# AiRyunn/BoT

Measured on AMD Instinct MI355X. Metric: edges/sec full-batch GAT fwd+bwd on ogbn-arxiv; achieved HBM GB/s vs peak, higher is better.
Workload: dtype f32

## Files before the change

bot_amd/_C.py:

```python
from __future__ import annotations

import ctypes
import os
from ctypes import c_char_p, c_double, c_float, c_int32, c_int64, c_uint64, c_void_p

import torch

_HERE = os.path.dirname(os.path.abspath(__file__))
LIB_PATH = os.environ.get("BOT_AMD_LIB") or os.path.join(_HERE, "lib", "libbot_gnn.so")
ABI_VERSION = 19

if not os.path.exists(LIB_PATH):
    raise ImportError(
        f"{LIB_PATH} is missing: build the gfx950 kernels first "
        "(`make -C bot_amd/csrc` or `python -c 'import __graft_entry__ as g; g.build()'`). "
        "bot_amd has no CPU / PyTorch fallback."
    )
_lib = ctypes.CDLL(LIB_PATH)

_P = c_void_p
_SIGS = {
    "bot_abi_version": (ctypes.c_int, []),
    "bot_last_error": (c_char_p, []),
    "bot_last_kernel": (c_char_p, []),
# ... 82 lines not shown
                                                 _P, _P, c_int64, c_int32, c_int32, _P]),
    "bot_bn_act_fwd_f32": (ctypes.c_int, [_P, c_int64, c_int64, c_int32, _P, _P, _P, _P, c_int32, c_float, c_uint64, _P, _P, c_int64, _P]),
    "bot_bn_act_bwd_reduce_f32": (ctypes.c_int, [_P, c_int64, _P, c_int64, c_int64, c_int32, _P, _P, _P, _P, c_int32, c_float,
                                                 c_uint64, _P, _P, _P, _P, _P]),
    "bot_bn_act_bwd_apply_f32": (ctypes.c_int, [_P, c_int64, _P, c_int64, c_int64, c_int32, _P, _P, _P, _P, c_int32, c_float,
                                                c_uint64, _P, _P, _P, c_double, _P, c_int64, _P, _P]),
    "bot_halves_tn_combine_f32": (ctypes.c_int, [_P, _P, c_int32, c_int32, c_int32, c_int32, _P, _P, _P, c_int64, _P]),
    "bot_halves_scale_from_slots2_f32": (ctypes.c_int, [_P, c_float, _P, c_float, _P, _P]),
    "bot_halves_tail_f16": (ctypes.c_int, [c_int64, c_int32, _P, _P, _P, _P, _P, c_int64, c_int32, _P]),
    "bot_spmm_dot_halves_fits": (ctypes.c_int, [_P, c_int64, c_int64, _P, c_int64, c_int64, c_int32, c_int32, _P, c_int64, c_int64, c_int32]),
    "bot_spmm_dot_halves_f16": (ctypes.c_int, [_P, _P, c_int64, c_int64, _P, c_int64, _P, _P, c_int64, _P, c_int64, c_int64, _P, _P, _P, c_int64, c_int64,
                                               c_int32, c_int32, _P, _P, c_int64, c_int64, c_int32, _P, _P, _P]),
    "bot_gemm_halves3_nt_bn_rows": (c_int32, [c_int64]),
    "bot_gemm_halves3_nt3_f32": (ctypes.c_int, [c_int64, c_int64, c_int64, _P, _P, c_int64, _P, _P, c_int64, c_int64, _P, c_int64, c_int64, c_int32, _P, c_int64,
                                                _P, c_int32, _P]),
    "bot_bn_act_bwd_reduce_partials_f32": (ctypes.c_int, [_P, c_int32, c_int32, _P, _P, _P]),
    "bot_bn_bwd_bound_partials_f32": (ctypes.c_int, [c_int32, _P, c_int32, _P, _P, c_double, _P, _P, _P, _P]),
    "bot_bn_bwd_partials_finish_f32": (ctypes.c_int, [_P, _P, c_int32, c_int32, _P, _P, c_int32, c_double, _P, _P, _P, _P]),
    "bot_gemm_halves3_nt2_f32": (ctypes.c_int, [c_int64, c_int64, c_int64, _P, _P, c_int64, _P, _P, c_int64, c_int64, _P, c_int64, c_int64, c_int32, _P, c_int64,
                                                c_int32, _P]),
    "bot_halves_split_frag_f16": (ctypes.c_int, [_P, c_int64, c_int64, c_int32, _P, _P, c_int32, _P]),
    "bot_gemm_halves3_tn2_f32": (ctypes.c_int, [c_int64, c_int64, c_int64, c_int64, c_int64, _P, _P, _P, c_int64, _P, c_int64, c_int64, _P, c_int64, c_int64, _P,
                                                c_int64, _P, c_int32, _P]),
    "bot_stream_create": (ctypes.c_int, [c_int32, _P]),
    "bot_gemm_halves3_nt_grouped2_f32": (ctypes.c_int, [c_int64, c_int64, _P, _P, _P, c_int64, c_int64, _P, c_int64, c_int64, _P, c_int64, c_int32, _P,
                                                        c_int32, _P, _P, c_int32, _P, _P, _P, _P, c_int32, c_int32, _P]),
    "bot_bn_stats_halves_partials_f32": (ctypes.c_int, [_P, _P, c_int32, _P, c_int64, c_int32, c_float, c_float, _P, _P, _P, _P, _P, _P, _P, c_float, _P, _P, _P]),
    "bot_absmax_slots": (c_int32, []),
    "bot_absmax_slots_f32": (ctypes.c_int, [_P, c_int64, c_int64, c_int32, _P, _P]),
    "bot_halves_scale_from_slots_f32": (ctypes.c_int, [_P, _P, _P]),
# ... 735 lines not shown
        sg = torch.empty(self.F, dtype=torch.float32, device=self.x.device)
        sgx = torch.empty(self.F, dtype=torch.float32, device=self.x.device)
        _check(_lib.bot_bn_bwd_partials_finish_f32(self.part.data_ptr(), self.pmax.data_ptr(), self.nblk, self.F, sg.data_ptr(), sgx.data_ptr(),
                                                   int(bool(batch_stats)), float(total_count), _ptr(self.weight), self.invstd.data_ptr(), slots.data_ptr(),
                                                   _stream()), "bn_bwd_partials_finish")
        return sg, sgx

    def bound(self, sum_g, sum_gx, total_count, slots):
        assert self.pmax is not None
        _dev(slots)
        _check(_lib.bot_bn_bwd_bound_partials_f32(self.F, self.pmax.data_ptr(), self.nblk, _ptr(sum_g), _ptr(sum_gx), float(total_count), _ptr(self.weight),
                                                  self.invstd.data_ptr(), slots.data_ptr(), _stream()), "bn_bwd_bound_partials")
        return slots


def gemm_halves3_nt(a, b, scale_a, scale_b, piece_a, piece_b, k, out=None, mode=0, a2_off=None, scale_a2=None, k_split=0, b_frag=False, n=None, bn=None):
    _dev(a, b, scale_a, scale_b, scale_a2)
    m = a.shape[0]
    if n is None:
        assert not b_frag
        n = b.shape[0]
    if out is None:
        out = torch.empty((m, n), dtype=torch.float32, device=a.device)
    st = None
    if bn is not None:
        if not bn.fits(m, n, k):
            raise BotKernelError("gemm_halves3_nt: this product cannot carry the BatchNorm-backward by-product (BnBwdStats.fits)")
        st = bn.struct()
    _check(_timed("gemm_halves", (m, n, 3 * k, 1), lambda: _lib.bot_gemm_halves3_nt3_f32(
        m, n, k, scale_a.data_ptr(), _ptr(scale_a2), int(k_split), scale_b.data_ptr(), a.data_ptr(), _ld(a), 2 * piece_a if a2_off is None else a2_off,
        b.data_ptr(), _ld(b), piece_b, int(bool(b_frag)), out.data_ptr(), _ld(out), ctypes.addressof(st) if st is not None else None, int(mode), _stream())),
        "gemm_halves3_nt")
    return out


def halves_split_frag(x, scale, piece):
    _dev(x, scale)
    x = _mat(x, "x")
    n, F = x.shape
    assert piece % 64 == 0 and piece >= F
    out = torch.empty((2 * ((n + 15) // 16) * (piece // 32), 512), dtype=torch.float16, device=x.device)
    _check(_lib.bot_halves_split_frag_f16(x.data_ptr(), x.stride(0), n, F, _ptr(scale), out.data_ptr(), piece, _stream()), "halves_split_frag")
    return out


def _table(rows, width):
# ... 600 lines not shown
```

bot_amd/csrc/halves3.hip:

```cpp
#include <hip/hip_fp16.h>

#include <stdlib.h>
#include <string.h>

#include <algorithm>
#include <type_traits>
#include <utility>

#include "common.h"

namespace bot {
namespace {

constexpr int BK = 32;

typedef _Float16 half8 __attribute__((ext_vector_type(8)));
typedef float f32x4 __attribute__((ext_vector_type(4)));

struct H3Args {
    const _Float16* A;
    const _Float16* B;
    const float* scale_a;
    const float* scale_b;
    float* C;
// ... 11 lines not shown
    float* stats_minmax;
    float* stats_pivot;
    int stats_F;
    const float* bnb_x;
    int64_t bnb_ldx;
    const float* bnb_mean;
    const float* bnb_invstd;
    const float* bnb_w;
    const float* bnb_b;
    int bnb_relu;
    float bnb_p;
    uint64_t bnb_seed;
    const uint64_t* bnb_seed_offset;
    float* bnb_part;
    float* bnb_pmax;
    int b_frag;
    int mode;
};

struct H3Group {
    int b_row0, n_valid;
    int a_off0, a_off1;
    int k_steps, pad;
    int64_t c_off;
};
constexpr int kMaxGroups = 12;
struct H3Groups {
    H3Group g[kMaxGroups];
    int k_seg;
};
// ... 267 lines not shown
}
template <int N, class F>
__device__ __forceinline__ void static_for(F& f) {
    static_for_impl(f, std::make_integer_sequence<int, N>{});
}

__device__ __forceinline__ half8 load16(const void* tile_base, uint32_t voff, int soff) {
#if defined(__HIP_DEVICE_COMPILE__)
    const __amdgpu_buffer_rsrc_t rsrc = __builtin_amdgcn_make_buffer_rsrc(const_cast<void*>(tile_base), 0, 0x7fffffff, 0x00020000);
    return __builtin_bit_cast(half8, __builtin_amdgcn_raw_buffer_load_b128(rsrc, voff, soff, 0));
#else
    return half8{};
#endif
}

template <bool GROUPED, bool BFRAG, bool BNB = false>
__device__ __forceinline__ void gemm_halves3_nt64_body(const H3Args& p, const H3Groups* groups) {
    static_assert(!(GROUPED && BNB), "the BatchNorm-backward by-product indexes the output columns of a plain launch");
    constexpr int BM = 256, BN = 256, kWaves = 8, MT = BM / 16, NT = BN / kWaves / 16;
    constexpr int kRow = 4 * BK;
    constexpr int kABytes = BM * kRow;
    constexpr int kStageBytes = 2 * kABytes, kStages = 2;
    constexpr int GA = BM / 8 / kWaves;
    static_assert(NT == 2 && GA == 4 && kRow == 128, "wave tile 256 x 32, 128-byte rows");
    __shared__ __attribute__((aligned(1024))) unsigned char lds[kStages * kStageBytes];
    const int tid = threadIdx.x, lane = tid & 63, w = __builtin_amdgcn_readfirstlane(tid >> 6);
    const int b = blockIdx.x, xcd = b & 7, j = b >> 3;
    const int tm = (j / p.tiles_n) * 8 + xcd, tn = j % p.tiles_n;
    if (tm >= p.tiles_m) return;
    const int m0 = tm * BM;
    int n0 = tn * BN, n_valid = p.N - n0, T = p.K / BK, a_off0 = 0, a_off1 = 0, k_seg = 0;
    int64_t c0 = n0;
    if constexpr (GROUPED) {
// ... 5 lines not shown

    const _Float16* tileA = p.A + (int64_t)m0 * p.lda;
    const _Float16* tileB = p.B + (int64_t)n0 * p.ldb;
    uint32_t offA[GA];
#pragma unroll
    for (int h = 0; h < GA; ++h) {
        const int row = (w + kWaves * h) * 8 + (lane >> 3);
        offA[h] = ((uint32_t)(min(m0 + row, p.M - 1) - m0) * (uint32_t)p.lda + (((lane & 7) ^ ((row >> 1) & 7)) * 8)) * 2;
    }
    const int a2b = p.a2_off * 2;
    auto issue_a = [&](int i, int stage, int it) {
        const int q = i / GA, h = i % GA;
        dma16(tileA, lds + stage * kStageBytes + q * kABytes + (w + kWaves * h) * 1024, offA[h],
              (GROUPED ? it * kRow + (2 * it < k_seg ? a_off0 : a_off1) : it * kRow) + q * a2b);
    };
    uint32_t offB[NT];
    int tileoff[NT];
    const int Tk = p.K / BK;
#pragma unroll
    for (int nt = 0; nt < NT; ++nt) {
        if constexpr (BFRAG) {
            offB[nt] = lane * 16;
            tileoff[nt] = min((n0 + w * (NT * 16) + nt * 16) >> 4, ((p.N + 15) >> 4) - 1) * Tk * 1024;
        } else {
            offB[nt] = ((uint32_t)(min(n0 + w * (NT * 16) + nt * 16 + (lane & 15), p.N - 1) - n0) * (uint32_t)p.ldb) * 2 + (lane >> 4) * 16;
            tileoff[nt] = 0;
        }
    }
    const int b2 = BFRAG ? ((p.N + 15) >> 4) * Tk * 1024 : p.b2_off * 2;
    const _Float16* baseB = BFRAG ? p.B : tileB;
// ... 106 lines not shown
    static_assert(32 * P * 4 <= kStages * kStageBytes / kWaves, "staging slab does not fit the wave's share of the LDS");
    float* stg = reinterpret_cast<float*>(lds + w * (kStages * kStageBytes / kWaves));
    const int q4 = (lane >> 4) * 4, l15 = lane & 15, l7 = lane & 7;
    const int col = w * (NT * 16) + l7 * 4;
    float cs[4] = {1.f, 1.f, 1.f, 1.f}, ch[4] = {0.f, 0.f, 0.f, 0.f};
    const bool affine = p.col_scale != nullptr || p.col_shift != nullptr;
    if (affine) {
#pragma unroll
        for (int e = 0; e < 4; ++e)
            if (col + e < n_valid) {
                if (p.col_scale) cs[e] = p.col_scale[c0 + col + e];
                if (p.col_shift) ch[e] = p.col_shift[c0 + col + e];
            }
    }
    float amax = 0.f;
    const bool stats = p.stats_part != nullptr;
    float st_s[4] = {0.f, 0.f, 0.f, 0.f}, st_q[4] = {0.f, 0.f, 0.f, 0.f}, st_mn[4], st_mx[4], piv[4] = {0.f, 0.f, 0.f, 0.f};
#pragma unroll
    for (int e = 0; e < 4; ++e) st_mn[e] = INFINITY, st_mx[e] = -INFINITY;
    float b_s[4] = {0.f, 0.f, 0.f, 0.f}, b_q[4] = {0.f, 0.f, 0.f, 0.f}, b_gm[4] = {0.f, 0.f, 0.f, 0.f}, b_xm[4] = {0.f, 0.f, 0.f, 0.f};
    float b_mu[4] = {0.f, 0.f, 0.f, 0.f}, b_is[4] = {0.f, 0.f, 0.f, 0.f}, b_sc[4] = {1.f, 1.f, 1.f, 1.f}, b_sh[4] = {0.f, 0.f, 0.f, 0.f};
    int b_nv = 0;
    bool b_wide = false;
    uint64_t b_seed = 0;
    int64_t b_nquad = 0;
    float b_keep = 1.f;
    if constexpr (BNB) {
        b_nv = max(0, min(4, n_valid - col));
#pragma unroll
        for (int e = 0; e < 4; ++e)
// ... 33 lines not shown
        }
    };
    load_x(std::integral_constant<int, 0>{});
    load_x(std::integral_constant<int, 1>{});
    auto do_pass = [&](auto pass_c) __attribute__((always_inline)) {
        constexpr int pass = decltype(pass_c)::value;
        load_x(std::integral_constant<int, pass + 2>{});
        const f32x4 (&b_x)[4] = b_ring[pass % 3];
#pragma unroll
        for (int mm = 0; mm < 2; ++mm)
#pragma unroll
            for (int nt = 0; nt < NT; ++nt) {
                const f32x4 v = acc[pass * 2 + mm][nt] * alpha;
                *reinterpret_cast<f32x4*>(stg + (mm * 16 + l15) * P + nt * 16 + q4) = v;
            }
#pragma unroll
        for (int i = 0; i < 4; ++i) {
            const int r = i * 8 + (lane >> 3);
            f32x4 v = *reinterpret_cast<const f32x4*>(stg + r * P + l7 * 4);
            const int row = m0 + pass * 32 + r;
            if (affine || p.relu) {
#pragma unroll
                for (int e = 0; e < 4; ++e) {
                    v[e] = fmaf(v[e], cs[e], ch[e]);
                    if (p.relu) v[e] = fmaxf(v[e], 0.f);
                }
            }
            if constexpr (pass == 0) {
                if (stats && i == 0) {
#pragma unroll
// ... 91 lines not shown
#pragma unroll
            for (int e = 0; e < 4; ++e)
                if (e < b_nv) ps[e] = b_s[e], ps[F + e] = b_q[e];
            if (p.bnb_pmax) {
                float* pm = p.bnb_pmax + ((int64_t)tm * 2) * F + c0 + col;
#pragma unroll
                for (int e = 0; e < 4; ++e)
                    if (e < b_nv) pm[e] = b_gm[e], pm[F + e] = b_xm[e];
            }
        }
    }
}

__global__ __launch_bounds__(512) void gemm_halves3_nt64_kernel(H3Args p) { gemm_halves3_nt64_body<false, false>(p, nullptr); }
__global__ __launch_bounds__(512) void gemm_halves3_nt64_frag_kernel(H3Args p) { gemm_halves3_nt64_body<false, true>(p, nullptr); }
__global__ __launch_bounds__(512) void gemm_halves3_nt64_grouped_kernel(H3Args p, H3Groups groups) { gemm_halves3_nt64_body<true, false>(p, &groups); }
__global__ __launch_bounds__(512) void gemm_halves3_nt64_bnb_kernel(H3Args p) { gemm_halves3_nt64_body<false, false, true>(p, nullptr); }
__global__ __launch_bounds__(512) void gemm_halves3_nt64_frag_bnb_kernel(H3Args p) { gemm_halves3_nt64_body<false, true, true>(p, nullptr); }

static bool nt64_wanted() {
    static const bool wanted = [] {
        const char* e = getenv("BOT_NT_KERNEL");
        return !(e && !strcmp(e, "128x64"));
    }();
    return wanted;
}

constexpr int TBK = 32;
constexpr int TT = 192;
constexpr int kTnSubA = TBK * 256, kTnSubB = TBK * 128;
// ... 312 lines not shown

extern "C" int bot_gemm_halves3_nt2_f32(int64_t m, int64_t n, int64_t k, const float* scale_a, const float* scale_a2, int64_t k_split, const float* scale_b,
                                        const uint16_t* A, int64_t lda, int64_t a2_off, const uint16_t* B, int64_t ldb, int64_t b2_off, int32_t b_layout,
                                        float* C, int64_t ldc, int32_t mode, bot_stream_t stream) {
    return bot_gemm_halves3_nt3_f32(m, n, k, scale_a, scale_a2, k_split, scale_b, A, lda, a2_off, B, ldb, b2_off, b_layout, C, ldc, nullptr, mode, stream);
}

extern "C" int32_t bot_gemm_halves3_nt_bn_rows(int64_t k) {
    using namespace bot;
    return (k > 0 && k % (2 * BK) == 0 && nt64_wanted()) ? 256 : 0;
}

extern "C" int bot_gemm_halves3_nt3_f32(int64_t m, int64_t n, int64_t k, const float* scale_a, const float* scale_a2, int64_t k_split, const float* scale_b,
                                        const uint16_t* A, int64_t lda, int64_t a2_off, const uint16_t* B, int64_t ldb, int64_t b2_off, int32_t b_layout,
                                        float* C, int64_t ldc, const bot_bn_bwd_stats_t* bn, int32_t mode, bot_stream_t stream) {
    using namespace bot;
    BOT_REQUIRE(bn == nullptr || (mode == 0 && bot_gemm_halves3_nt_bn_rows(k) == 256), -1,
                "gemm_halves3_nt3: the BatchNorm-backward by-product rides on the 256 x 32 form (mode 0, k a multiple of 64, BOT_NT_KERNEL not 128x64)");
    BOT_REQUIRE(bn == nullptr || (bn->x && bn->mean && bn->invstd && bn->part), -1, "gemm_halves3_nt3: bn->x, mean, invstd and part must be set");
    BOT_REQUIRE(bn == nullptr || (n % 2 == 0 && bn->ldx >= n && bn->ldx % 2 == 0 && aligned(bn->x, 8) && bn->p >= 0.f && bn->p < 1.f), -1,
                "gemm_halves3_nt3: the by-product needs an even n (= the BatchNorm width), 8-byte aligned x rows of pitch >= n and p in [0, 1)");
    BOT_REQUIRE(b_layout == 0 || (b_layout == 1 && mode == 0 && k % 64 == 0), -1,
                "gemm_halves3_nt2: b_layout 1 (fragment-major B, bot_halves_split_frag_f16 with piece = k) needs mode 0 and k a multiple of 64");
    BOT_REQUIRE(scale_a2 == nullptr || (k_split > 0 && k_split < k && k_split % BK == 0), -1,
                "gemm_halves3_nt2: the second scale starts at a column that is a positive multiple of %d below k (got %lld of %lld)", BK, (long long)k_split,
                (long long)k);
    BOT_REQUIRE(m > 0 && n > 0 && k > 0 && k % BK == 0, -1, "gemm_halves3_nt: m, n > 0 and k a positive multiple of %d (got %lld %lld %lld)", BK,
                (long long)m, (long long)n, (long long)k);
    BOT_REQUIRE(scale_a && scale_b && A && B && C, -1, "gemm_halves3_nt: null pointer");
    BOT_REQUIRE(aligned(A, 16) && aligned(B, 16) && lda % 8 == 0 && ldb % 8 == 0 && a2_off % 8 == 0 && b2_off % 8 == 0, -1,
                "gemm_halves3_nt: operands, row pitches and piece offsets must be 16-byte aligned");
    BOT_REQUIRE(a2_off + k <= lda && (b_layout == 1 || b2_off + k <= ldb) && ldc >= n && m < (1ll << 31) - 256 && n < (1ll << 31) - 256, -1, "gemm_halves3_nt: bad pitches");
    BOT_REQUIRE(b_layout == 0 || ((n + 15) / 16) * (k / 32) * 2048 < (1ll << 31), -1, "gemm_halves3_nt2: fragment-major B exceeds the 2 GiB a buffer descriptor spans");
    H3Args p;
    p.A = reinterpret_cast<const _Float16*>(A), p.B = reinterpret_cast<const _Float16*>(B), p.scale_a = scale_a, p.scale_b = scale_b, p.C = C;
    p.lda = lda, p.ldb = ldb, p.ldc = ldc, p.M = (int)m, p.N = (int)n, p.K = (int)k, p.a2_off = (int)a2_off, p.b2_off = (int)b2_off;
    p.tiles_m = p.tiles_n = 0;
    p.col_scale = p.col_shift = nullptr, p.relu = 0, p.absmax = nullptr;
    p.scale_a2 = scale_a2, p.k2 = scale_a2 ? (int)(k_split / BK) : -1;
    p.b_frag = b_layout;
    p.stats_part = p.stats_minmax = nullptr, p.stats_pivot = nullptr, p.stats_F = 0;
    p.bnb_x = nullptr, p.bnb_ldx = 0, p.bnb_mean = p.bnb_invstd = p.bnb_w = p.bnb_b = nullptr, p.bnb_relu = 0, p.bnb_p = 0.f, p.bnb_seed = 0;
    p.bnb_seed_offset = nullptr, p.bnb_part = p.bnb_pmax = nullptr;
    p.mode = mode;
    const bool force_128x64 = (mode & 1024) != 0;
    mode &= ~1024;
    p.mode = mode;
    if (bn) {
        p.bnb_x = bn->x, p.bnb_ldx = bn->ldx, p.bnb_mean = bn->mean, p.bnb_invstd = bn->invstd, p.bnb_w = bn->weight, p.bnb_b = bn->bias;
        p.bnb_relu = bn->relu, p.bnb_p = bn->p, p.bnb_seed = bn->seed, p.bnb_seed_offset = bn->seed_offset, p.bnb_part = bn->part, p.bnb_pmax = bn->pmax;
        p.tiles_m = (int)((m + 255) / 256), p.tiles_n = (int)((n + 255) / 256);
        set_kernel(b_layout ? "bot::gemm_halves3_nt64_frag_bnb_kernel" : "bot::gemm_halves3_nt64_bnb_kernel");
        if (b_layout) hipLaunchKernelGGL(gemm_halves3_nt64_frag_bnb_kernel, dim3(((p.tiles_m + 7) / 8) * 8 * p.tiles_n), dim3(512), 0, (hipStream_t)stream, p);
        else hipLaunchKernelGGL(gemm_halves3_nt64_bnb_kernel, dim3(((p.tiles_m + 7) / 8) * 8 * p.tiles_n), dim3(512), 0, (hipStream_t)stream, p);
    } else if (mode == 0 && !force_128x64 && nt64_wanted() && (k / BK) % 2 == 0) {
        p.tiles_m = (int)((m + 255) / 256), p.tiles_n = (int)((n + 255) / 256);
        set_kernel(b_layout ? "bot::gemm_halves3_nt64_frag_kernel" : "bot::gemm_halves3_nt64_kernel");
        if (b_layout) hipLaunchKernelGGL(gemm_halves3_nt64_frag_kernel, dim3(((p.tiles_m + 7) / 8) * 8 * p.tiles_n), dim3(512), 0, (hipStream_t)stream, p);
        else hipLaunchKernelGGL(gemm_halves3_nt64_kernel, dim3(((p.tiles_m + 7) / 8) * 8 * p.tiles_n), dim3(512), 0, (hipStream_t)stream, p);
    } else if (b_layout) {
        BOT_REQUIRE(false, -1, "gemm_halves3_nt2: a fragment-major B is read by the 256 x 32 form only (BOT_NT_KERNEL=128x64 / mode bit 1024 exclude it)");
    } else if (mode & 32) {
        set_kernel("bot::gemm_halves3_nt_kernel<256,256,2,4,plain>");
        launch_h3<256, 256, 2, 4, false, true>(p, m, n, (hipStream_t)stream);
    } else if (mode) {
        set_kernel("bot::gemm_halves3_nt_kernel<256,256,2,4,pipelined,ablate>");
        launch_h3<256, 256, 2, 4, true, true>(p, m, n, (hipStream_t)stream);
    } else {
        set_kernel("bot::gemm_halves3_nt_kernel<256,256,2,4,pipelined>");
// ... 17 lines not shown
                                                int32_t mode, bot_stream_t stream) {
    using namespace bot;
    BOT_REQUIRE((stats_part == nullptr) == (stats_minmax == nullptr) && (stats_part == nullptr) == (stats_pivot == nullptr) && (stats_part == nullptr || stats_F >= 1), -1,
                "gemm_halves3_nt_grouped2: stats_part, stats_minmax and stats_pivot go together (stats_F = their row width)");
    BOT_REQUIRE(m > 0 && b_rows > 0 && n_groups >= 1 && n_groups <= kMaxGroups && k_seg >= 0, -1, "gemm_halves3_nt_grouped: m, b_rows > 0, 1 .. %d groups (got %lld %lld %d)",
                kMaxGroups, (long long)m, (long long)b_rows, n_groups);
    BOT_REQUIRE(scale_a && scale_b && A && B && C && groups, -1, "gemm_halves3_nt_grouped: null pointer");
    BOT_REQUIRE(aligned(A, 16) && aligned(B, 16) && lda % 8 == 0 && ldb % 8 == 0 && a2_off % 8 == 0 && b2_off % 8 == 0, -1,
                "gemm_halves3_nt_grouped: operands, row pitches and piece offsets must be 16-byte aligned");
    BOT_REQUIRE(m < (1ll << 31) - 256 && b_rows < (1ll << 31) - 256 && 256 * lda * 2 < (1ll << 31) && 256 * ldb * 2 < (1ll << 31), -1, "gemm_halves3_nt_grouped: bad sizes");
    H3Args p;
    p.A = reinterpret_cast<const _Float16*>(A), p.B = reinterpret_cast<const _Float16*>(B), p.scale_a = scale_a, p.scale_b = scale_b, p.C = C;
    p.lda = lda, p.ldb = ldb, p.ldc = ldc, p.M = (int)m, p.N = (int)b_rows, p.K = 0, p.a2_off = (int)a2_off, p.b2_off = (int)b2_off;
    p.mode = 0;
    p.scale_a2 = nullptr, p.k2 = -1, p.b_frag = 0;
    p.stats_part = stats_part, p.stats_minmax = stats_minmax, p.stats_pivot = stats_pivot, p.stats_F = stats_F;
    p.col_scale = col_scale, p.col_shift = col_shift, p.relu = relu, p.absmax = absmax_slots;
    H3Groups g;
    g.k_seg = k_seg;
    for (int i = 0; i < n_groups; ++i) {
        const int64_t* d = groups + 6 * i;
        const int64_t k_steps = d[4], a_hi = std::max(k_seg > 0 ? d[2] + 32 * std::min<int64_t>(k_seg, k_steps) : 0, k_steps > k_seg ? d[3] + 32 * k_steps : 0);
        BOT_REQUIRE(d[0] >= 0 && d[0] < b_rows && d[1] >= 1 && d[1] <= 256 && k_steps >= 1 && d[2] >= 0 && d[3] >= 0 && d[2] % 8 == 0 && d[3] % 8 == 0 && d[5] >= 0, -1,
                    "gemm_halves3_nt_grouped: group %d: b_row0=%lld n_valid=%lld a_col0=%lld a_col1=%lld k_steps=%lld c_off=%lld", i, (long long)d[0],
                    (long long)d[1], (long long)d[2], (long long)d[3], (long long)d[4], (long long)d[5]);
        BOT_REQUIRE(a_hi + a2_off <= lda && 32 * k_steps + b2_off <= ldb && 32 * k_steps <= b2_off, -1,
                    "gemm_halves3_nt_grouped: group %d reads past a row (A columns to %lld + %lld of %lld, B columns to %lld + %lld of %lld)", i, (long long)a_hi,
                    (long long)a2_off, (long long)lda, (long long)(32 * k_steps), (long long)b2_off, (long long)ldb);
        g.g[i] = H3Group{(int)d[0], (int)d[1], (int)d[2] * 2, (int)d[3] * 2, (int)k_steps, 0, d[5]};
    }
// ... 125 lines not shown
```

bot_amd/gemm.py:

```python
from __future__ import annotations

import os
import weakref

import torch

from . import _C

MODE = os.environ.get("BOT_GEMM", "halves")
NT_KERNEL = os.environ.get("BOT_GEMM_NT", "halves3")
TN_KERNEL = os.environ.get("BOT_GEMM_TN", "halves3")
LEFT_NODUP = NT_KERNEL == "halves3" and TN_KERNEL == "halves3" and os.environ.get("BOT_HALVES_DUP", "0") != "1"
NODUP_MIN_PIECE = int(os.environ.get("BOT_NODUP_MIN_PIECE", "256"))
TN_MIN_OUT = 512 * 1024
NT_MIN_COLS = 192
LINEAR_BLOCKS = os.environ.get("BOT_LINEAR_BLOCKS", "1") != "0"
FORCE = False
MIN_ROWS = 8192
PIECE_ALIGN = 64
SHIFT = 2048.0
CHUNK_ROWS = 8192


def enabled(x) -> bool:
# ... 129 lines not shown
    return split(x, order)


def epilogue_piece(F: int, x) -> int | None:
    if MODE != "halves" or not (FORCE or (x.is_cuda and x.shape[0] >= MIN_ROWS)) or F % 2 or x.stride(0) % 2:
        return None
    return (F + PIECE_ALIGN - 1) // PIECE_ALIGN * PIECE_ALIGN


def _alpha(a: Halves, b: Halves, n=None):
    if n is None:
        return a.scale[1:] * b.scale[1:]
    return torch.mul(a.scale[1:].expand(n), b.scale[1:].expand(n))


def mm_nt(a: Halves, b: Halves, out=None, link: BnLink | None = None):
    assert a.left and b.order in (1, 3) and a.F == b.F and a.piece == b.piece
    if NT_KERNEL == "halves3" and (b.order == 3 or b.n >= NT_MIN_COLS or a.order == 2):
        st = link.stats_for(a.n, b.n, a.piece) if (link is not None and out is None) else None
        res = _C.gemm_halves3_nt(a.buf, b.buf, a.scale, b.scale, a.piece, b.piece, a.piece, out=out, a2_off=a.h2_off, b_frag=b.order == 3, n=b.n, bn=st)
        if st is not None:
            link.deliver(st, res)
        return res
    assert a.order == 0 and b.order == 1
    return _C.gemm_halves(a.buf, b.buf, _alpha(a, b, b.n), trans_b=True, out=out)


TN_NARROW = os.environ.get("BOT_GEMM_TN_NARROW", "1") != "0"
_TN_TILES = {}


def _tn_tiles(K: int, P: int):
    key = (K, P)
    if key not in _TN_TILES:
        pt = 128 if (P + 127) // 128 * ((K + 191) // 192) <= 16 else 192
        tiles = [(192 * i, min(192, K - 192 * i), pt * j, min(pt, P - pt * j), 192 * i * P + pt * j, P, 0)
                 for i in range((K + 191) // 192) for j in range((P + pt - 1) // pt)]
        _TN_TILES[key] = tiles if len(tiles) <= 16 else None
    return _TN_TILES[key]
# ... 120 lines not shown
```

bot_amd/nn/fused.py:

```python
from __future__ import annotations

import os
from types import SimpleNamespace

import torch
import torch.nn as nn
import torch.nn.functional as F

from .. import _C, gemm, halo, side
from ..graph import take_rows
from ..ops import bn_epilogue_forward, bn_epilogue_sums, new_dropout_seed, stats_partials_for


ABSMAX_BYPRODUCT = os.environ.get("BOT_ABSMAX_BYPRODUCT", "1") != "0"
SKIP_Y = os.environ.get("BOT_SKIP_Y", "1") != "0"
HANDLES = 0
SKINNY = os.environ.get("BOT_SKINNY", "1") != "0"
FORCE = False
CALLS = 0
AGG_CALLS = 0
L0_CALLS = 0


def can_fuse(conv, norm, activation, graph, training, stack_residual) -> bool:
    epilogue_ok = norm is None or (isinstance(norm, nn.BatchNorm1d) and activation in (F.relu, torch.relu) and not stack_residual)
    return (epilogue_ok and hasattr(conv, "fc") and not (conv._use_symmetric_norm and graph.halo is not None)
            and conv._activation is None
            and not (training and (conv.edge_drop > 0 or conv.feat_drop.p > 0)) and conv._out_feats <= 256)


def sym_scales(graph):
    from . import _graph_cache, degree_norm
    c = _graph_cache(graph)
    if "sym_scales" not in c:
        csc = graph.csc
# ... 172 lines not shown
    c = 2 * B
    return (DOUT_DIRECT and ctx.halves is not None and has_res and epi is not None and not ctx.overlap and g.halo is None and not ctx.sym
            and g.number_of_dst_nodes() == h.shape[0]
            and HD % 2 == 0 and H >= 2 and c % 32 == 0 and P % 64 == 0 and gemm.left_order(P) == 2
            and gemm.NT_KERNEL == "halves3" and gemm.TN_KERNEL == "halves3" and (ctx.halves[2] * P >= gemm.TN_MIN_OUT or gemm.FORCE or FORCE) and not epi.sync)


class _GATHidden(torch.autograd.Function):
    @staticmethod
    def forward(ctx, h, Wcat, bn_w, bn_b, graph, bn, H, D, has_res, has_er, slope, attn_p, drop_p, bn_training, kp, sym, y_needed=True):
        N, HD = graph.number_of_dst_nodes(), H * D
        csc = graph.csc
        ctx.cfg, ctx.graph = (H, D, has_res, has_er, slope), graph
        ctx.sym = sym
        ctx.kp = kp
        xh = None
        if gemm.enabled(h):
            xh = gemm.take(h, 0)
            ws = gemm.split_right(Wcat.t().contiguous() if kp else Wcat)
            ctx.wscale = ws.scale
            ctx.xscale = xh.scale
            out = gemm.mm_nt(xh, ws)
        else:
            out = torch.mm(h, Wcat) if kp else torch.mm(h, Wcat.t())
        ctx.halves = None if xh is None else (xh.n, xh.F, xh.piece, xh.order)
        ctx.bn_link = None if xh is None else xh.bn_link
        hk = h if xh is None else xh.buf
        B = block_width(HD)
        c = 2 * B if has_res else B
        ext = None
        ctx.overlap = halo.enabled(graph) and not sym
        if ctx.overlap:
            global OVERLAP_CALLS
            OVERLAP_CALLS += 1
            plan, sp = graph.halo, graph.halo_split
            el_own = out[:, c:c + H].contiguous()
            el_halo, _, _ = _ship_rows(plan, el_own)
# ... 5 lines not shown
            a, a_d = _C.gat_attn_fwd(csc, el, er, None, None, None, slope, H, None, ctx.zs, drop=ctx.adrop or (0.0, 0))
            res = out[:, B:B + HD].unflatten(1, (H, D)) if has_res else None
            x3 = _C.spmm(sp["csc_own"], out[:, :HD].unflatten(1, (H, D)), a_d, sp["csc_own_pos"], addend=res)
            work.wait()
            del send_keep
            if sp["csc_halo"].nnz:
                _C.spmm(sp["csc_halo"], ft_halo.unflatten(1, (H, D)), a_d, sp["csc_halo_pos"], out=x3, addend=x3)
            return _finish_forward(ctx, x3.view(N, HD), bn, bn_w, bn_b, bn_training, drop_p, y_needed,
                                   h=hk, Wcat=Wcat, table=out, el=el, er=er, a=a, a_d=a_d, ft_halo=ft_halo)
        if graph.halo is not None:
            ext = _extend_forward(graph, out, HD, H, c)
            ft = ext[:, :HD].unflatten(1, (H, D))
            el = ext[:, HD:HD + H].contiguous()
        else:
            ft = out[:, :HD].unflatten(1, (H, D))
            el = out[:, c:c + H].contiguous()
        er = out[:N, c + H:c + 2 * H].contiguous() if has_er else None
        if sym:
            s_out, w_e = sym_scales(graph)
            el = el * s_out.unsqueeze(1)
        ctx.zs = _C.zsign_buffer(csc, H, slope)
        ctx.adrop = (attn_p, new_dropout_seed(attn_p)) if attn_p > 0 else None
        a, a_d = _C.gat_attn_fwd(csc, el, er, None, None, None, slope, H, None, ctx.zs, drop=ctx.adrop or (0.0, 0))
        if sym:
            a_d = a_d * w_e
        res = out[:N, B:B + HD].unflatten(1, (H, D)) if has_res else None
        if HD % 4 and bn is not None and sweep_is_row_kernel(graph, H, D):
            xbuf = torch.empty((N, (HD + 3) // 4 * 4), dtype=out.dtype, device=out.device)
            x = xbuf[:, :HD]
            _C.spmm(csc, ft, a_d, None, out=x.unflatten(1, (H, D)), addend=res)
        else:
            x = _C.spmm(csc, ft, a_d, None, addend=res).view(N, HD)
# ... 674 lines not shown
```

include/bot_gnn.h:

```cpp
#ifndef BOT_GNN_H
#define BOT_GNN_H

#include <stdint.h>

#ifdef __cplusplus
extern "C" {
#endif

#define BOT_ABI_VERSION 19

#define BOT_E_NULL (-1)
#define BOT_E_RANGE (-2)
#define BOT_E_ALIGN (-3)
#define BOT_E_PLAN (-4)

typedef void* bot_stream_t;

int bot_abi_version(void);
const char* bot_last_error(void);
int bot_stream_create(int32_t high_priority, bot_stream_t* out);
const char* bot_last_kernel(void);
int bot_debug_abort_trace(const char* path_host);

int bot_row_plan_size_host(const int32_t* indptr_host, int64_t n_rows, int32_t chunk,
// ... 238 lines not shown
    const float* mean;
    const float* invstd;
    const float* weight;
    const float* bias;
    int32_t relu;
    float p;
    uint64_t seed;
    const uint64_t* seed_offset;
    float* part;
    float* pmax;
} bot_bn_bwd_stats_t;
int32_t bot_gemm_halves3_nt_bn_rows(int64_t k);
int bot_gemm_halves3_nt3_f32(int64_t m, int64_t n, int64_t k, const float* scale_a, const float* scale_a2, int64_t k_split, const float* scale_b,
                             const uint16_t* A, int64_t lda, int64_t a2_off, const uint16_t* B, int64_t ldb, int64_t b2_off, int32_t b_layout, float* C,
                             int64_t ldc, const bot_bn_bwd_stats_t* bn, int32_t mode, bot_stream_t stream);
int bot_bn_act_bwd_reduce_partials_f32(const float* part, int32_t nblk, int32_t F, float* sum_g, float* sum_gx, bot_stream_t stream);
int bot_bn_bwd_bound_partials_f32(int32_t F, const float* pmax, int32_t nblk, const float* sum_g, const float* sum_gx, double total_count,
                                  const float* weight, const float* invstd, uint32_t* absmax_slots, bot_stream_t stream);
int bot_bn_bwd_partials_finish_f32(const float* part, const float* pmax, int32_t nblk, int32_t F, float* sum_g, float* sum_gx, int32_t batch_stats,
                                   double total_count, const float* weight, const float* invstd, uint32_t* absmax_slots, bot_stream_t stream);
int bot_halves_split_frag_f16(const float* x, int64_t ldx, int64_t n, int32_t F, const float* scale, uint16_t* out, int32_t piece, bot_stream_t stream);
int bot_gemm_halves3_tn2_f32(int64_t n_rows, int64_t k, int64_t p, int64_t kp, int64_t pp, const float* scale_x, const float* scale_d, const float* scale_d2,
                             int64_t p_split, const uint16_t* X, int64_t ldx, int64_t x2_off, const uint16_t* D, int64_t ldd, int64_t d2_off, float* out,
                             int64_t ldo, float* workspace, int32_t mode, bot_stream_t stream);

int bot_gemm_halves3_nt_grouped_f32(int64_t m, int64_t b_rows, const float* scale_a, const float* scale_b, const uint16_t* A, int64_t lda,
                                    int64_t a2_off, const uint16_t* B, int64_t ldb, int64_t b2_off, float* C, int64_t ldc, int32_t n_groups,
                                    const int64_t* groups, int32_t k_seg, const float* col_scale, const float* col_shift, int32_t relu,
                                    uint32_t* absmax_slots, int32_t mode, bot_stream_t stream);
int bot_gemm_halves3_nt_grouped2_f32(int64_t m, int64_t b_rows, const float* scale_a, const float* scale_b, const uint16_t* A, int64_t lda,
// ... 47 lines not shown
```

Baseline: 235.7 million.

## Emit GAT attention score columns as contiguous by-products from the projection GEMM epilogue

The projection GEMM gains an auxiliary epilogue. From the staged tile it writes the el/er attention-score columns straight into separate contiguous [N,H] buffers, so the later strided .contiguous() copy kernels are no longer needed. The kernel also adds an early-exit path for waves whose column slab lies wholly beyond the valid output: they only issue the shared A-tile loads and barriers and skip the MFMA work. The cost is a serial per-lane store loop in the epilogue and a new kernel variant, and the path is used only when the score columns fit inside one 32-column slab.

```diff
diff --git a/bot_amd/_C.py b/bot_amd/_C.py
--- a/bot_amd/_C.py
+++ b/bot_amd/_C.py
@@ -120,6 +120,8 @@
     "bot_gemm_halves3_nt_bn_rows": (c_int32, [c_int64]),
     "bot_gemm_halves3_nt3_f32": (ctypes.c_int, [c_int64, c_int64, c_int64, _P, _P, c_int64, _P, _P, c_int64, c_int64, _P, c_int64, c_int64, c_int32, _P, c_int64,
                                                 _P, c_int32, _P]),
+    "bot_gemm_halves3_nt4_f32": (ctypes.c_int, [c_int64, c_int64, c_int64, _P, _P, c_int64, _P, _P, c_int64, c_int64, _P, c_int64, c_int64, c_int32, _P, c_int64,
+                                                _P, _P, c_int64, c_int32, c_int32, _P, c_int64, c_int32, c_int32, _P]),
     "bot_bn_act_bwd_reduce_partials_f32": (ctypes.c_int, [_P, c_int32, c_int32, _P, _P, _P]),
     "bot_bn_bwd_bound_partials_f32": (ctypes.c_int, [c_int32, _P, c_int32, _P, _P, c_double, _P, _P, _P, _P]),
     "bot_bn_bwd_partials_finish_f32": (ctypes.c_int, [_P, _P, c_int32, c_int32, _P, _P, c_int32, c_double, _P, _P, _P, _P]),
@@ -885,8 +887,9 @@
         return slots
 
 
-def gemm_halves3_nt(a, b, scale_a, scale_b, piece_a, piece_b, k, out=None, mode=0, a2_off=None, scale_a2=None, k_split=0, b_frag=False, n=None, bn=None):
-    _dev(a, b, scale_a, scale_b, scale_a2)
+def gemm_halves3_nt(a, b, scale_a, scale_b, piece_a, piece_b, k, out=None, mode=0, a2_off=None, scale_a2=None, k_split=0, b_frag=False, n=None, bn=None,
+                    aux=None, aux_col0=0, aux2=None):
+    _dev(a, b, scale_a, scale_b, scale_a2, aux, aux2)
     m = a.shape[0]
     if n is None:
         assert not b_frag
@@ -898,9 +901,16 @@
         if not bn.fits(m, n, k):
             raise BotKernelError("gemm_halves3_nt: this product cannot carry the BatchNorm-backward by-product (BnBwdStats.fits)")
         st = bn.struct()
-    _check(_timed("gemm_halves", (m, n, 3 * k, 1), lambda: _lib.bot_gemm_halves3_nt3_f32(
+    for t in (aux, aux2):
+        if t is not None and (t.dtype != torch.float32 or t.dim() != 2 or t.shape[0] != m or t.stride(1) != 1):
+            raise BotKernelError(f"gemm_halves3_nt: aux must be float32 [{m}, cols] with unit column stride, got {tuple(t.shape)} {t.dtype}")
+    if aux2 is not None and aux is None:
+        raise BotKernelError("gemm_halves3_nt: aux2 without aux")
+    _check(_timed("gemm_halves", (m, n, 3 * k, 1), lambda: _lib.bot_gemm_halves3_nt4_f32(
         m, n, k, scale_a.data_ptr(), _ptr(scale_a2), int(k_split), scale_b.data_ptr(), a.data_ptr(), _ld(a), 2 * piece_a if a2_off is None else a2_off,
-        b.data_ptr(), _ld(b), piece_b, int(bool(b_frag)), out.data_ptr(), _ld(out), ctypes.addressof(st) if st is not None else None, int(mode), _stream())),
+        b.data_ptr(), _ld(b), piece_b, int(bool(b_frag)), out.data_ptr(), _ld(out), ctypes.addressof(st) if st is not None else None,
+        _ptr(aux), _ld(aux) if aux is not None else 0, int(aux_col0), aux.shape[1] if aux is not None else 0,
+        _ptr(aux2), _ld(aux2) if aux2 is not None else 0, aux2.shape[1] if aux2 is not None else 0, int(mode), _stream())),
         "gemm_halves3_nt")
     return out
 
diff --git a/bot_amd/csrc/halves3.hip b/bot_amd/csrc/halves3.hip
--- a/bot_amd/csrc/halves3.hip
+++ b/bot_amd/csrc/halves3.hip
@@ -49,6 +49,10 @@
     const uint64_t* bnb_seed_offset;
     float* bnb_part;
     float* bnb_pmax;
+    float* aux;
+    float* aux2;
+    int64_t aux_ld, aux2_ld;
+    int aux_c0, aux_n, aux2_n;
     int b_frag;
     int mode;
 };
@@ -346,9 +350,10 @@
 #endif
 }
 
-template <bool GROUPED, bool BFRAG, bool BNB = false>
+template <bool GROUPED, bool BFRAG, bool BNB = false, bool AUX = false>
 __device__ __forceinline__ void gemm_halves3_nt64_body(const H3Args& p, const H3Groups* groups) {
     static_assert(!(GROUPED && BNB), "the BatchNorm-backward by-product indexes the output columns of a plain launch");
+    static_assert(!AUX || (!GROUPED && !BNB), "the auxiliary columns ride on the plain launches (no affine epilogue: what is staged is what is stored)");
     constexpr int BM = 256, BN = 256, kWaves = 8, MT = BM / 16, NT = BN / kWaves / 16;
     constexpr int kRow = 4 * BK;
     constexpr int kABytes = BM * kRow;
@@ -384,6 +389,22 @@
         dma16(tileA, lds + stage * kStageBytes + q * kABytes + (w + kWaves * h) * 1024, offA[h],
               (GROUPED ? it * kRow + (2 * it < k_seg ? a_off0 : a_off1) : it * kRow) + q * a2b);
     };
+    if (w * (NT * 16) >= n_valid) {
+#pragma unroll
+        for (int i = 0; i < 2 * GA; ++i) issue_a(i, 0, 0);
+        asm volatile("s_waitcnt vmcnt(0)" ::: "memory");
+        __builtin_amdgcn_s_barrier();
+        for (int it = 0; it < T2; ++it) {
+            if (it + 1 < T2) {
+#pragma unroll
+                for (int i = 0; i < 2 * GA; ++i) issue_a(i, (it & 1) ^ 1, it + 1);
+            }
+            asm volatile("s_waitcnt vmcnt(0)" ::: "memory");
+            __builtin_amdgcn_s_barrier();
+        }
+        __builtin_amdgcn_s_barrier();
+        return;
+    }
     uint32_t offB[NT];
     int tileoff[NT];
     const int Tk = p.K / BK;
@@ -520,6 +541,8 @@
             }
     }
     float amax = 0.f;
+    const int aux_s0 = AUX ? p.aux_c0 - (n0 + w * (NT * 16)) : 0;
+    const bool aux_mine = AUX && aux_s0 >= 0 && aux_s0 < NT * 16;
     const bool stats = p.stats_part != nullptr;
     float st_s[4] = {0.f, 0.f, 0.f, 0.f}, st_q[4] = {0.f, 0.f, 0.f, 0.f}, st_mn[4], st_mx[4], piv[4] = {0.f, 0.f, 0.f, 0.f};
 #pragma unroll
@@ -583,6 +606,18 @@
                 const f32x4 v = acc[pass * 2 + mm][nt] * alpha;
                 *reinterpret_cast<f32x4*>(stg + (mm * 16 + l15) * P + nt * 16 + q4) = v;
             }
+        if constexpr (AUX) {
+            if (aux_mine && lane < 32) {
+                const int row = m0 + pass * 32 + lane;
+                if (row < p.M) {
+                    const float* sv = stg + lane * P + aux_s0;
+#pragma nounroll
+                    for (int jj = 0; jj < p.aux_n; ++jj) p.aux[(int64_t)row * p.aux_ld + jj] = sv[jj];
+#pragma nounroll
+                    for (int jj = 0; jj < p.aux2_n; ++jj) p.aux2[(int64_t)row * p.aux2_ld + jj] = sv[p.aux_n + jj];
+                }
+            }
+        }
 #pragma unroll
         for (int i = 0; i < 4; ++i) {
             const int r = i * 8 + (lane >> 3);
@@ -704,6 +739,8 @@
 
 __global__ __launch_bounds__(512) void gemm_halves3_nt64_kernel(H3Args p) { gemm_halves3_nt64_body<false, false>(p, nullptr); }
 __global__ __launch_bounds__(512) void gemm_halves3_nt64_frag_kernel(H3Args p) { gemm_halves3_nt64_body<false, true>(p, nullptr); }
+__global__ __launch_bounds__(512) void gemm_halves3_nt64_aux_kernel(H3Args p) { gemm_halves3_nt64_body<false, false, false, true>(p, nullptr); }
+__global__ __launch_bounds__(512) void gemm_halves3_nt64_frag_aux_kernel(H3Args p) { gemm_halves3_nt64_body<false, true, false, true>(p, nullptr); }
 __global__ __launch_bounds__(512) void gemm_halves3_nt64_grouped_kernel(H3Args p, H3Groups groups) { gemm_halves3_nt64_body<true, false>(p, &groups); }
 __global__ __launch_bounds__(512) void gemm_halves3_nt64_bnb_kernel(H3Args p) { gemm_halves3_nt64_body<false, false, true>(p, nullptr); }
 __global__ __launch_bounds__(512) void gemm_halves3_nt64_frag_bnb_kernel(H3Args p) { gemm_halves3_nt64_body<false, true, true>(p, nullptr); }
@@ -1046,7 +1083,23 @@
 extern "C" int bot_gemm_halves3_nt3_f32(int64_t m, int64_t n, int64_t k, const float* scale_a, const float* scale_a2, int64_t k_split, const float* scale_b,
                                         const uint16_t* A, int64_t lda, int64_t a2_off, const uint16_t* B, int64_t ldb, int64_t b2_off, int32_t b_layout,
                                         float* C, int64_t ldc, const bot_bn_bwd_stats_t* bn, int32_t mode, bot_stream_t stream) {
+    return bot_gemm_halves3_nt4_f32(m, n, k, scale_a, scale_a2, k_split, scale_b, A, lda, a2_off, B, ldb, b2_off, b_layout, C, ldc, bn, nullptr, 0, 0, 0, nullptr,
+                                    0, 0, mode, stream);
+}
+
+extern "C" int bot_gemm_halves3_nt4_f32(int64_t m, int64_t n, int64_t k, const float* scale_a, const float* scale_a2, int64_t k_split, const float* scale_b,
+                                        const uint16_t* A, int64_t lda, int64_t a2_off, const uint16_t* B, int64_t ldb, int64_t b2_off, int32_t b_layout,
+                                        float* C, int64_t ldc, const bot_bn_bwd_stats_t* bn, float* aux, int64_t aux_ld, int32_t aux_col0, int32_t aux_cols,
+                                        float* aux2, int64_t aux2_ld, int32_t aux2_cols, int32_t mode, bot_stream_t stream) {
     using namespace bot;
+    BOT_REQUIRE(aux != nullptr || (aux2 == nullptr && aux_cols == 0 && aux2_cols == 0), -1, "gemm_halves3_nt4: aux2 / column counts without aux");
+    BOT_REQUIRE(aux == nullptr || (mode == 0 && bn == nullptr && bot_gemm_halves3_nt_bn_rows(k) == 256), -1,
+                "gemm_halves3_nt4: the auxiliary columns ride on the 256 x 32 form (mode 0, k a multiple of 64, BOT_NT_KERNEL not 128x64), without bn");
+    BOT_REQUIRE(aux == nullptr || (aux_cols >= 1 && aux2_cols >= 0 && (aux2 != nullptr) == (aux2_cols > 0) && aux_cols + aux2_cols <= 8 && aux_col0 >= 0 &&
+                                   (int64_t)aux_col0 + aux_cols + aux2_cols <= n && aux_col0 / 32 == (aux_col0 + aux_cols + aux2_cols - 1) / 32 &&
+                                   aux_ld >= aux_cols && (aux2 == nullptr || aux2_ld >= aux2_cols)), -1,
+                "gemm_halves3_nt4: 1 .. 8 auxiliary columns inside the product and inside one 32-column slab (got %d + %d from column %d of %lld)", aux_cols,
+                aux2_cols, aux_col0, (long long)n);
     BOT_REQUIRE(bn == nullptr || (mode == 0 && bot_gemm_halves3_nt_bn_rows(k) == 256), -1,
                 "gemm_halves3_nt3: the BatchNorm-backward by-product rides on the 256 x 32 form (mode 0, k a multiple of 64, BOT_NT_KERNEL not 128x64)");
     BOT_REQUIRE(bn == nullptr || (bn->x && bn->mean && bn->invstd && bn->part), -1, "gemm_halves3_nt3: bn->x, mean, invstd and part must be set");
@@ -1074,6 +1127,7 @@
     p.stats_part = p.stats_minmax = nullptr, p.stats_pivot = nullptr, p.stats_F = 0;
     p.bnb_x = nullptr, p.bnb_ldx = 0, p.bnb_mean = p.bnb_invstd = p.bnb_w = p.bnb_b = nullptr, p.bnb_relu = 0, p.bnb_p = 0.f, p.bnb_seed = 0;
     p.bnb_seed_offset = nullptr, p.bnb_part = p.bnb_pmax = nullptr;
+    p.aux = aux, p.aux2 = aux2, p.aux_ld = aux_ld, p.aux2_ld = aux2_ld, p.aux_c0 = aux_col0, p.aux_n = aux_cols, p.aux2_n = aux2_cols;
     p.mode = mode;
     const bool force_128x64 = (mode & 1024) != 0;
     mode &= ~1024;
@@ -1085,6 +1139,11 @@
         set_kernel(b_layout ? "bot::gemm_halves3_nt64_frag_bnb_kernel" : "bot::gemm_halves3_nt64_bnb_kernel");
         if (b_layout) hipLaunchKernelGGL(gemm_halves3_nt64_frag_bnb_kernel, dim3(((p.tiles_m + 7) / 8) * 8 * p.tiles_n), dim3(512), 0, (hipStream_t)stream, p);
         else hipLaunchKernelGGL(gemm_halves3_nt64_bnb_kernel, dim3(((p.tiles_m + 7) / 8) * 8 * p.tiles_n), dim3(512), 0, (hipStream_t)stream, p);
+    } else if (aux) {
+        p.tiles_m = (int)((m + 255) / 256), p.tiles_n = (int)((n + 255) / 256);
+        set_kernel(b_layout ? "bot::gemm_halves3_nt64_frag_aux_kernel" : "bot::gemm_halves3_nt64_aux_kernel");
+        if (b_layout) hipLaunchKernelGGL(gemm_halves3_nt64_frag_aux_kernel, dim3(((p.tiles_m + 7) / 8) * 8 * p.tiles_n), dim3(512), 0, (hipStream_t)stream, p);
+        else hipLaunchKernelGGL(gemm_halves3_nt64_aux_kernel, dim3(((p.tiles_m + 7) / 8) * 8 * p.tiles_n), dim3(512), 0, (hipStream_t)stream, p);
     } else if (mode == 0 && !force_128x64 && nt64_wanted() && (k / BK) % 2 == 0) {
         p.tiles_m = (int)((m + 255) / 256), p.tiles_n = (int)((n + 255) / 256);
         set_kernel(b_layout ? "bot::gemm_halves3_nt64_frag_kernel" : "bot::gemm_halves3_nt64_kernel");
@@ -1132,6 +1191,7 @@
     p.lda = lda, p.ldb = ldb, p.ldc = ldc, p.M = (int)m, p.N = (int)b_rows, p.K = 0, p.a2_off = (int)a2_off, p.b2_off = (int)b2_off;
     p.mode = 0;
     p.scale_a2 = nullptr, p.k2 = -1, p.b_frag = 0;
+    p.aux = p.aux2 = nullptr, p.aux_ld = p.aux2_ld = 0, p.aux_c0 = p.aux_n = p.aux2_n = 0;
     p.stats_part = stats_part, p.stats_minmax = stats_minmax, p.stats_pivot = stats_pivot, p.stats_F = stats_F;
     p.col_scale = col_scale, p.col_shift = col_shift, p.relu = relu, p.absmax = absmax_slots;
     H3Groups g;
diff --git a/bot_amd/gemm.py b/bot_amd/gemm.py
--- a/bot_amd/gemm.py
+++ b/bot_amd/gemm.py
@@ -167,15 +167,25 @@
     return torch.mul(a.scale[1:].expand(n), b.scale[1:].expand(n))
 
 
-def mm_nt(a: Halves, b: Halves, out=None, link: BnLink | None = None):
+def _nt_halves3(a: Halves, b: Halves) -> bool:
+    return NT_KERNEL == "halves3" and (b.order == 3 or b.n >= NT_MIN_COLS or a.order == 2)
+
+
+def nt_carries_aux(a: Halves, b: Halves, col0: int, cols: int) -> bool:
+    return (_nt_halves3(a, b) and int(_C._lib.bot_gemm_halves3_nt_bn_rows(a.piece)) == 256 and 1 <= cols <= 8 and col0 + cols <= b.n
+            and col0 // 32 == (col0 + cols - 1) // 32)
+
+
+def mm_nt(a: Halves, b: Halves, out=None, link: BnLink | None = None, aux=None):
     assert a.left and b.order in (1, 3) and a.F == b.F and a.piece == b.piece
-    if NT_KERNEL == "halves3" and (b.order == 3 or b.n >= NT_MIN_COLS or a.order == 2):
+    if _nt_halves3(a, b):
         st = link.stats_for(a.n, b.n, a.piece) if (link is not None and out is None) else None
-        res = _C.gemm_halves3_nt(a.buf, b.buf, a.scale, b.scale, a.piece, b.piece, a.piece, out=out, a2_off=a.h2_off, b_frag=b.order == 3, n=b.n, bn=st)
+        kw = {} if aux is None else dict(aux_col0=aux[0], aux=aux[1], aux2=aux[2])
+        res = _C.gemm_halves3_nt(a.buf, b.buf, a.scale, b.scale, a.piece, b.piece, a.piece, out=out, a2_off=a.h2_off, b_frag=b.order == 3, n=b.n, bn=st, **kw)
         if st is not None:
             link.deliver(st, res)
         return res
-    assert a.order == 0 and b.order == 1
+    assert a.order == 0 and b.order == 1 and aux is None
     return _C.gemm_halves(a.buf, b.buf, _alpha(a, b, b.n), trans_b=True, out=out)
 
 
diff --git a/bot_amd/nn/fused.py b/bot_amd/nn/fused.py
--- a/bot_amd/nn/fused.py
+++ b/bot_amd/nn/fused.py
@@ -13,12 +13,14 @@
 
 
 ABSMAX_BYPRODUCT = os.environ.get("BOT_ABSMAX_BYPRODUCT", "1") != "0"
+SCORE_AUX = os.environ.get("BOT_SCORE_AUX", "1") != "0"
 SKIP_Y = os.environ.get("BOT_SKIP_Y", "1") != "0"
 HANDLES = 0
 SKINNY = os.environ.get("BOT_SKINNY", "1") != "0"
 FORCE = False
 CALLS = 0
 AGG_CALLS = 0
+SCORE_AUX_CALLS = 0
 L0_CALLS = 0
 
 
@@ -221,13 +223,18 @@
         ctx.cfg, ctx.graph = (H, D, has_res, has_er, slope), graph
         ctx.sym = sym
         ctx.kp = kp
-        xh = None
+        xh = score = None
         if gemm.enabled(h):
             xh = gemm.take(h, 0)
             ws = gemm.split_right(Wcat.t().contiguous() if kp else Wcat)
             ctx.wscale = ws.scale
             ctx.xscale = xh.scale
-            out = gemm.mm_nt(xh, ws)
+            c_ = (2 if has_res else 1) * block_width(HD)
+            if SCORE_AUX and h.is_cuda and graph.halo is None and not sym and gemm.nt_carries_aux(xh, ws, c_, 2 * H if has_er else H):
+                score = (h.new_empty((xh.n, H), dtype=torch.float32), h.new_empty((xh.n, H), dtype=torch.float32) if has_er else None)
+                global SCORE_AUX_CALLS
+                SCORE_AUX_CALLS += 1
+            out = gemm.mm_nt(xh, ws, aux=None if score is None else (c_, score[0], score[1]))
         else:
             out = torch.mm(h, Wcat) if kp else torch.mm(h, Wcat.t())
         ctx.halves = None if xh is None else (xh.n, xh.F, xh.piece, xh.order)
@@ -263,8 +270,11 @@
             el = ext[:, HD:HD + H].contiguous()
         else:
             ft = out[:, :HD].unflatten(1, (H, D))
-            el = out[:, c:c + H].contiguous()
-        er = out[:N, c + H:c + 2 * H].contiguous() if has_er else None
+            el = score[0] if score is not None else out[:, c:c + H].contiguous()
+        if score is not None:
+            er = score[1][:N] if has_er else None
+        else:
+            er = out[:N, c + H:c + 2 * H].contiguous() if has_er else None
         if sym:
             s_out, w_e = sym_scales(graph)
             el = el * s_out.unsqueeze(1)
diff --git a/include/bot_gnn.h b/include/bot_gnn.h
--- a/include/bot_gnn.h
+++ b/include/bot_gnn.h
@@ -276,6 +276,10 @@
 int bot_gemm_halves3_nt3_f32(int64_t m, int64_t n, int64_t k, const float* scale_a, const float* scale_a2, int64_t k_split, const float* scale_b,
                              const uint16_t* A, int64_t lda, int64_t a2_off, const uint16_t* B, int64_t ldb, int64_t b2_off, int32_t b_layout, float* C,
                              int64_t ldc, const bot_bn_bwd_stats_t* bn, int32_t mode, bot_stream_t stream);
+int bot_gemm_halves3_nt4_f32(int64_t m, int64_t n, int64_t k, const float* scale_a, const float* scale_a2, int64_t k_split, const float* scale_b,
+                             const uint16_t* A, int64_t lda, int64_t a2_off, const uint16_t* B, int64_t ldb, int64_t b2_off, int32_t b_layout, float* C,
+                             int64_t ldc, const bot_bn_bwd_stats_t* bn, float* aux, int64_t aux_ld, int32_t aux_col0, int32_t aux_cols, float* aux2,
+                             int64_t aux2_ld, int32_t aux2_cols, int32_t mode, bot_stream_t stream);
 int bot_bn_act_bwd_reduce_partials_f32(const float* part, int32_t nblk, int32_t F, float* sum_g, float* sum_gx, bot_stream_t stream);
 int bot_bn_bwd_bound_partials_f32(int32_t F, const float* pmax, int32_t nblk, const float* sum_g, const float* sum_gx, double total_count,
                                   const float* weight, const float* invstd, uint32_t* absmax_slots, bot_stream_t stream);
```

Result: no change. 236.7 million (median of 6 runs) (+0.4%).
